# Razyehuda/Hyperparameter-GNN_unfolded-D-ADMM-main

Measured on AMD Instinct MI355X. Metric: ADMM-iters/sec (node), batch=4096 P=5 n=256 K=25; final-iter MSE vs ref, higher is better.
Workload: dtype f32; 1 GPU; DLASSO_unfolded.forward B=4096/GPU P=5 n=256 m=64 K=25 ER(p=0.5) shared graph; global_batch=4096, P=5, n=256, m=64, K=25, parallelism=batch-sharded dp1

## Files before the change

### hyperparameter-gnn_unfolded-d-admm-main_amd/csrc/dadmm_abi.cpp

```cpp

#include <hip/hip_runtime.h>
#include <stdarg.h>
#include <stdio.h>
#include <stdlib.h>
#include <string.h>

#include "../../include/dadmm.h"
#include "dadmm_internal.h"

namespace {

thread_local char g_err[512] = "";

int fail(int code, const char* fmt, ...) {
    va_list ap;
    va_start(ap, fmt);
    vsnprintf(g_err, sizeof(g_err), fmt, ap);
    va_end(ap);
    return code;
}

int ok() {
    g_err[0] = '\0';
    return DADMM_OK;
}

int hip_rc(hipError_t e, const char* what) {
    if (e != hipSuccess) return fail(DADMM_EHIP, "%s: %s", what, hipGetErrorString(e));
    return ok();
}

bool aligned16(const void* p) { return ((uintptr_t)p & 15u) == 0; }
template <typename... T>
bool all_aligned16(const T*... p) { return (... && aligned16(p)); }
template <typename... T>
bool any_null(const T*... p) { return (... || (p == nullptr)); }

int check_dims(const dadmm_dims* d) {
    if (d == nullptr) return fail(DADMM_EINVAL, "dims is NULL");
    if (d->B < 0 || d->P < 1 || d->m < 1 || d->n < 1 || d->K < 0)
        return fail(DADMM_EINVAL, "bad dims B=%d P=%d m=%d n=%d K=%d", d->B, d->P, d->m, d->n,
                    d->K);
    if (d->P > 255) return fail(DADMM_EINVAL, "P=%d > 255 agents does not fit the uint8 visit-list ids", d->P);
    if (d->variant != DADMM_VARIANT_UNFOLDED && d->variant != DADMM_VARIANT_GNN)
        return fail(DADMM_EINVAL, "unknown variant %d", d->variant);
    if (d->hyp_rows != 1 && d->hyp_rows != d->P)
        return fail(DADMM_EINVAL, "hyp_rows=%d must be 1 ('same') or P=%d ('diff')", d->hyp_rows,
                    d->P);
    if (d->graph_shared != 0 && d->graph_shared != 1)
        return fail(DADMM_EINVAL, "graph_shared must be 0 or 1");
    return DADMM_OK;
}

int n_pad_of(const dadmm_dims* d) { return 64 * dadmm::fused_nt(d->n); }
int m_pad_of(const dadmm_dims* d) { return dadmm::m_pad_of(d->m); }

int check_m(const dadmm_dims* d) {
    if (d->m > dadmm::M_MAX)
        return fail(DADMM_EUNSUPPORTED, "m=%d > %d rows per agent", d->m, dadmm::M_MAX);
    return DADMM_OK;
}

size_t align256(size_t x) { return (x + 255) & ~(size_t)255; }

int check_scratch256(const void* scratch) {
    if (((uintptr_t)scratch & 255u) != 0) return fail(DADMM_EINVAL, "scratch must be 256-byte aligned");
    return DADMM_OK;
}
int check_n4(const dadmm_dims* d, const char* who = "") {
    if ((d->n & 3) != 0) return fail(DADMM_EUNSUPPORTED, "n=%d: %sneeds n %% 4 == 0 (zero-pad n)", d->n, who);
    return DADMM_OK;
}
bool iterate_fits(const dadmm_dims* d) { return (size_t)d->B * d->P * d->n * 4 < ((size_t)1 << 31); }
int check_iterate(const dadmm_dims* d) {
    if (!iterate_fits(d)) return fail(DADMM_EUNSUPPORTED, "B*P*n*4 >= 2^31 bytes per iterate (split the batch)");
    return DADMM_OK;
}
int zero_dhyp(const dadmm_dims* d, float* dhyp, void* stream) {
    return hip_rc(hipMemsetAsync(dhyp, 0, sizeof(float) * (size_t)d->K * d->hyp_rows * 4, (hipStream_t)stream),
                  "memset");
}

template <typename Args>
void fill_args(Args& a, const dadmm_dims* d, const void* op) {
    a.A = (const float*)op;
    a.At = op ? a.A + (size_t)d->P * m_pad_of(d) * n_pad_of(d) : nullptr;
    a.B = d->B;
    a.m = d->m;
    a.n = d->n;
    a.K = d->K;
    a.hyp_rows = d->hyp_rows;
    a.variant = d->variant;
}
template <typename Args>
void fill_args_padded(Args& a, const dadmm_dims* d, const void* op) {
    fill_args(a, d, op);
    a.P = d->P;
    a.m_pad = m_pad_of(d);
    a.n_pad = n_pad_of(d);
    a.graph_shared = d->graph_shared;
}

}

extern "C" {

int dadmm_abi_version(void) { return DADMM_ABI_VERSION; }

const char* dadmm_last_error(void) { return g_err; }

size_t dadmm_operator_bytes(const dadmm_dims* d) {
    if (check_dims(d) != DADMM_OK) return 0;
    if (check_m(d) != DADMM_OK) return 0;
    return 2 * sizeof(float) * (size_t)d->P * m_pad_of(d) * (size_t)n_pad_of(d);
}

int dadmm_prepare_operator(const dadmm_dims* d, const float* A, void* op, void* stream) {
    int rc = check_dims(d);
    if (rc) return rc;
    if (A == nullptr || op == nullptr) return fail(DADMM_EINVAL, "A/op is NULL");
    if (!aligned16(op)) return fail(DADMM_EINVAL, "op workspace must be 16-byte aligned");
    if ((rc = check_m(d)) != DADMM_OK) return rc;
    const int np = n_pad_of(d);
    float* Apad = (float*)op;
    float* Atpad = Apad + (size_t)d->P * m_pad_of(d) * np;
    return hip_rc(dadmm::launch_prepare(A, Apad, Atpad, d->P, d->m, d->n, np, (hipStream_t)stream), "prepare launch");
}

}

namespace {

int check_fused_shape(const dadmm_dims* d, const uint32_t* nbr_order, int* graph, int* nt) {
    if (d->m > dadmm::M_PAD)
        return fail(DADMM_EUNSUPPORTED, "m=%d > %d rows per agent: not a fused shape", d->m,
                    dadmm::M_PAD);
    int rc = check_n4(d, "the fused kernel ");
    if (rc || (rc = check_iterate(d)) != DADMM_OK) return rc;
    if (nbr_order != nullptr && d->graph_shared)
        return fail(DADMM_EINVAL, "nbr_order needs per-sample graphs (graph_shared = 0)");
    if (nbr_order != nullptr && d->P > 8)
        return fail(DADMM_EINVAL, "nbr_order packs 4-bit agent ids: P <= 8");
    *nt = dadmm::fused_nt(d->n);
    *graph = d->graph_shared ? dadmm::GRAPH_SHARED
                             : (nbr_order ? dadmm::GRAPH_ORDERED : dadmm::GRAPH_LANE);
    return DADMM_OK;
}

void fill_fused(dadmm::FusedArgs& a, const dadmm_dims* d, const void* op, const float* b, const uint64_t* nbr,
                const uint32_t* nbr_order, const float* deg, const float* hyp, const float* y0, const float* U0,
                const float* d0, float* Y, float* U_out, int32_t* status) {
    fill_args(a, d, op);
    a.b = b;
    a.nbr = nbr;
    a.nbr_order = nbr_order;
    a.deg = deg;
    a.hyp = hyp;
    a.y0 = y0;
    a.U0 = U0;
    a.d0 = d0;
    a.Y = Y;
    a.U_out = U_out;
    a.status = status;
    a.Grec = nullptr;
    a.Urec = nullptr;
}

int forward_impl(const dadmm_dims* d, const void* op, const float* b, const uint64_t* nbr,
                 const uint32_t* nbr_order, const float* deg, const float* hyp, const float* y0,
                 const float* U0, const float* d0, float* Y, float* Grec, float* Urec,
                 float* U_out, int32_t* status, void* stream, bool rec) {
    int rc = check_dims(d);
    if (rc) return rc;
    if (d->B == 0 || d->K == 0) return ok();
    if (rec && (any_null(Grec, Urec) || !all_aligned16(Grec, Urec)))
        return fail(DADMM_EINVAL, "Grec and Urec must be non-NULL and 16-byte aligned");
    if (any_null(op, b, nbr, deg, hyp, y0, U0, d0, Y)) return fail(DADMM_EINVAL, "a required pointer is NULL");
    if (!aligned16(op)) return fail(DADMM_EINVAL, "op workspace must be 16-byte aligned");
    if (!all_aligned16(Y, y0, U0, d0, U_out))
        return fail(DADMM_EINVAL, "Y, y0, U0, d0 and U_out must be 16-byte aligned");
    int graph = 0, nt = 0;
    if ((rc = check_fused_shape(d, nbr_order, &graph, &nt)) != DADMM_OK) return rc;
    dadmm::fused_fn_ptr fn = rec ? dadmm::find_fused_rec(d->P, nt, graph) : dadmm::find_fused(d->P, nt, graph);
    if (fn == nullptr)
        return fail(DADMM_EUNSUPPORTED, "no fused kernel for P=%d n=%d (n_pad=%d)", d->P, d->n,
                    64 * nt);
    dadmm::FusedArgs a;
    fill_fused(a, d, op, b, nbr, nbr_order, deg, hyp, y0, U0, d0, Y, U_out, status);
    a.Grec = Grec;
    a.Urec = Urec;
    return hip_rc(fn(a, (hipStream_t)stream), "fused launch");
}

}

extern "C" {

int dadmm_forward(const dadmm_dims* d, const void* op, const float* b, const uint64_t* nbr,
                  const uint32_t* nbr_order, const float* deg, const float* hyp, const float* y0,
                  const float* U0, const float* d0, float* Y, float* U_out, int32_t* status,
                  void* stream) {
    return forward_impl(d, op, b, nbr, nbr_order, deg, hyp, y0, U0, d0, Y, nullptr, nullptr, U_out,
                        status, stream, false);
}

int dadmm_forward_record(const dadmm_dims* d, const void* op, const float* b, const uint64_t* nbr,
                         const uint32_t* nbr_order, const float* deg, const float* hyp,
                         const float* y0, const float* U0, const float* d0, float* Y, float* Grec,
                         float* Urec, float* U_out, int32_t* status, void* stream) {
    return forward_impl(d, op, b, nbr, nbr_order, deg, hyp, y0, U0, d0, Y, Grec, Urec, U_out,
                        status, stream, true);
}

namespace {
int device_cus() {
    int dev = 0, cus = 0;
    if (hipGetDevice(&dev) != hipSuccess ||
        hipDeviceGetAttribute(&cus, hipDeviceAttributeMultiprocessorCount, dev) != hipSuccess || cus < 1)
        cus = 256;
    return cus;
}
struct SplitPlan {
    int nt = 0, slices = 0, groups = 0, tiles = 0;
    size_t flag_bytes = 0, bytes = 0;
};
SplitPlan split_plan(const dadmm_dims* d) {
    SplitPlan sp;
    if (d == nullptr || d->B <= 0 || d->K <= 0 || d->P < 1 || d->P > 6 || d->m < 1 ||
        d->m > dadmm::M_PAD || d->n < 1 || (d->n & 3) != 0 || d->hyp_rows < 1)
        return sp;
    if (!iterate_fits(d)) return sp;
    const int nt = dadmm::fused_nt(d->n);
    if (nt != 2 && nt != 4) return sp;
    const int cus = device_cus();
    const int tiles = (d->B + dadmm::BT - 1) / dadmm::BT;
    if (2 * tiles > cus) return sp;
    const int S = 64 * nt / dadmm::SPLIT_COLS;
    int groups = cus / S;
    groups = groups < tiles ? groups : tiles;
    if (groups < 1) return sp;
    sp.nt = nt;
    sp.slices = S;
    sp.groups = groups;
    sp.tiles = tiles;
    sp.flag_bytes = ((size_t)groups * d->P * 4 * S * 4 + 4 + 255) / 256 * 256;
    sp.bytes = (size_t)groups * 2 * d->P * 4 * S * 1024;
    return sp;
}

int split_impl(const dadmm_dims* d, const void* op, const float* b, const uint64_t* nbr,
               const uint32_t* nbr_order, const float* deg, const float* hyp, const float* y0,
               const float* U0, const float* d0, float* Y, float* Grec, float* Urec, float* U_out,
               int32_t* status, void* flags, void* scratch, void* stream, bool rec) {
    int rc = check_dims(d);
    if (rc) return rc;
    if (d->B == 0 || d->K == 0) return ok();
    if (rec && (any_null(Grec, Urec) || !all_aligned16(Grec, Urec)))
        return fail(DADMM_EINVAL, "Grec and Urec must be non-NULL and 16-byte aligned");
    if (any_null(op, b, nbr, deg, hyp, y0, U0, d0, Y, flags, scratch))
        return fail(DADMM_EINVAL, "a required pointer is NULL");
    if (!all_aligned16(op, Y, y0, U0, d0, flags, scratch, U_out))
        return fail(DADMM_EINVAL, "op, Y, y0, U0, d0, U_out, flags and scratch must be 16-byte aligned");
    int graph = 0, nt = 0;
    if ((rc = check_fused_shape(d, nbr_order, &graph, &nt)) != DADMM_OK) return rc;
    const SplitPlan sp = split_plan(d);
    if (sp.groups == 0)
        return fail(DADMM_EUNSUPPORTED, "the column-split forward does not serve B=%d P=%d n=%d "
                    "(n_pad 128 or 256, P <= 6, ceil(B/16) <= CUs/2)", d->B, d->P, d->n);
    dadmm::split_fn_ptr fn = rec ? dadmm::find_split_rec(d->P, nt, graph) : dadmm::find_split(d->P, nt, graph);
    if (fn == nullptr)
        return fail(DADMM_EUNSUPPORTED, "no split kernel for P=%d n_pad=%d", d->P, 64 * nt);
    dadmm::SplitArgs sa;
    fill_fused(sa.f, d, op, b, nbr, nbr_order, deg, hyp, y0, U0, d0, Y, U_out, status);
    sa.f.Grec = Grec;
    sa.f.Urec = Urec;
    sa.xflag = (uint32_t*)flags;
    sa.xbuf = (float*)scratch;
    sa.groups = sp.groups;
    sa.tiles = sp.tiles;
    sa.spin_ticks = 20000000ull;
    return hip_rc(fn(sa, (hipStream_t)stream), "split launch");
}
}

size_t dadmm_split_scratch_bytes(const dadmm_dims* d) {
    if (d == nullptr || check_dims(d) != DADMM_OK) return 0;
    return split_plan(d).bytes;
}

size_t dadmm_split_flag_bytes(const dadmm_dims* d) {
    if (d == nullptr || check_dims(d) != DADMM_OK) return 0;
    return split_plan(d).flag_bytes;
}

int dadmm_forward_split(const dadmm_dims* d, const void* op, const float* b, const uint64_t* nbr,
                        const uint32_t* nbr_order, const float* deg, const float* hyp,
                        const float* y0, const float* U0, const float* d0, float* Y, float* U_out,
                        int32_t* status, void* flags, void* scratch, void* stream) {
    return split_impl(d, op, b, nbr, nbr_order, deg, hyp, y0, U0, d0, Y, nullptr, nullptr, U_out, status,
                      flags, scratch, stream, false);
}

int dadmm_forward_split_record(const dadmm_dims* d, const void* op, const float* b, const uint64_t* nbr,
                               const uint32_t* nbr_order, const float* deg, const float* hyp,
                               const float* y0, const float* U0, const float* d0, float* Y, float* Grec,
                               float* Urec, float* U_out, int32_t* status, void* flags, void* scratch,
                               void* stream) {
    return split_impl(d, op, b, nbr, nbr_order, deg, hyp, y0, U0, d0, Y, Grec, Urec, U_out, status,
                      flags, scratch, stream, true);
}

size_t dadmm_backward_scratch_bytes(const dadmm_dims* d) {
    if (check_dims(d) != DADMM_OK) return 0;
    const size_t nwg = ((size_t)d->B + dadmm::BT - 1) / dadmm::BT;
    const size_t bytes = sizeof(float) * nwg * (size_t)d->K * d->P * 4;
    return bytes > 0 ? bytes : 16;
}

int dadmm_backward(const dadmm_dims* d, const void* op, const uint64_t* nbr,
                   const uint32_t* nbr_order, const float* deg, const float* hyp, const float* y0,
                   const float* d0, const float* Y, const float* Grec, const float* Urec,
                   const float* gY, float* dhyp, void* scratch, void* stream) {
    int rc = check_dims(d);
    if (rc) return rc;
    if (d->K == 0) return ok();
    if (!dhyp) return fail(DADMM_EINVAL, "dhyp is NULL");
    if (d->B == 0) return zero_dhyp(d, dhyp, stream);
    if (any_null(op, nbr, deg, hyp, y0, d0, Y, Grec, Urec, gY, scratch))
        return fail(DADMM_EINVAL, "a required pointer is NULL");
    if (!all_aligned16(op, Y, y0, d0, Grec, Urec, gY, scratch))
        return fail(DADMM_EINVAL, "op, Y, y0, d0, Grec, Urec, gY and scratch must be 16-byte aligned");
    int graph = 0, nt = 0;
    if ((rc = check_fused_shape(d, nbr_order, &graph, &nt)) != DADMM_OK) return rc;
    dadmm::backward_fn_ptr fn = dadmm::find_backward(d->P, nt, graph);
    if (fn == nullptr)
        return fail(DADMM_EUNSUPPORTED, "no adjoint kernel for P=%d n=%d (n_pad=%d)", d->P, d->n,
                    64 * nt);
    dadmm::BackwardArgs a;
    fill_args(a, d, op);
    a.nbr = nbr;
    a.nbr_order = nbr_order;
    a.deg = deg;
    a.hyp = hyp;
    a.y0 = y0;
    a.d0 = d0;
    a.Y = Y;
    a.Grec = Grec;
    a.Urec = Urec;
    a.gY = gY;
    a.partial = (float*)scratch;
    if ((rc = hip_rc(fn(a, (hipStream_t)stream), "adjoint launch")) != DADMM_OK) return rc;
    const int nwg = (d->B + dadmm::BT - 1) / dadmm::BT;
    return hip_rc(dadmm::launch_backward_reduce(a.partial, dhyp, nwg, d->K, d->P, d->hyp_rows, (hipStream_t)stream),
                  "adjoint reduce launch");
}

size_t dadmm_adjoint_scratch_bytes(const dadmm_dims* d) {
    if (check_dims(d) != DADMM_OK) return 0;
    const size_t state = align256(sizeof(float) * (size_t)d->B * d->P * d->n);
    const size_t part = sizeof(float) * (size_t)dadmm::adjoint_workgroups(d->B, d->n, d->P) * d->K * d->P * 4;
    return 3 * state + align256(part > 0 ? part : 16);
}

int dadmm_adjoint(const dadmm_dims* d, const void* op, const int32_t* visit_ptr,
                  const uint8_t* visit_q, const float* deg, const float* hyp, const float* y0,
                  const float* d0, const float* Y, const float* Grec, const float* Urec,
                  const float* gY, float* dhyp, void* scratch, void* stream) {
    int rc = check_dims(d);
    if (rc) return rc;
    if (d->K == 0) return ok();
    if (!dhyp) return fail(DADMM_EINVAL, "dhyp is NULL");
    if (d->B == 0) return zero_dhyp(d, dhyp, stream);
    if (any_null(op, visit_ptr, visit_q, deg, hyp, y0, d0, Y, Grec, Urec, gY, scratch))
        return fail(DADMM_EINVAL, "a required pointer is NULL");
    if (!all_aligned16(op, Y, y0, d0, Grec, Urec, gY))
        return fail(DADMM_EINVAL, "op, Y, y0, d0, Grec, Urec and gY must be 16-byte aligned");
    if ((rc = check_scratch256(scratch)) != DADMM_OK || (rc = check_m(d)) != DADMM_OK ||
        (rc = check_n4(d)) != DADMM_OK || (rc = check_iterate(d)) != DADMM_OK)
        return rc;
    if (dadmm::adjoint_lds_bytes(d->P) > 160 * 1024 || dadmm::gnn_gram_lds(m_pad_of(d)) > 160 * 1024)
        return fail(DADMM_EUNSUPPORTED, "P=%d / m=%d: the adjoint's LDS tiles do not fit", d->P, d->m);
    const size_t state = align256(sizeof(float) * (size_t)d->B * d->P * d->n);
    char* base = (char*)scratch;
    dadmm::AdjArgs a{};
    fill_args_padded(a, d, op);
    a.vptr = visit_ptr;
    a.vq = visit_q;
    a.deg = deg;
    a.hyp = hyp;
    a.y0 = y0;
    a.d0 = d0;
    a.Y = Y;
    a.Grec = Grec;
    a.Urec = Urec;
    a.gY = gY;
    a.yb = (float*)base;
    a.Ub = (float*)(base + state);
    a.Gb = (float*)(base + 2 * state);
    a.partial = (float*)(base + 3 * state);
    return hip_rc(dadmm::launch_adjoint(a, dhyp, (hipStream_t)stream), "adjoint launch");
}

namespace {

int gnn_common(const dadmm_dims* d, const void* op, dadmm::GnnArgs* a) {
    int rc = check_dims(d);
    if (rc || (rc = check_m(d)) != DADMM_OK || (rc = check_n4(d)) != DADMM_OK ||
        (rc = check_iterate(d)) != DADMM_OK)
        return rc;
    *a = dadmm::GnnArgs{};
    fill_args_padded(*a, d, op);
    return DADMM_OK;
}

}

size_t dadmm_gnn_flag_bytes(int32_t K) {
    return K < 0 ? 0 : (size_t)GNN_FLAG_WORDS(K) * 4;
}

int dadmm_gnn_begin(const dadmm_dims* d, const void* op, const float* b, const float* y0,
                    const float* U0, float* Atb, int32_t* flags, void* stream) {
    dadmm::GnnArgs a;
    int rc = gnn_common(d, op, &a);
    if (rc) return rc;
    if (!flags) return fail(DADMM_EINVAL, "flags is NULL");
    if (d->B == 0) return hip_rc(dadmm::gnn_launch_zero(flags, GNN_FLAG_WORDS(d->K), (hipStream_t)stream), "zero launch");
    if (any_null(op, b, y0, U0, Atb)) return fail(DADMM_EINVAL, "a required pointer is NULL");
    if (!all_aligned16(op, y0, U0, Atb))
        return fail(DADMM_EINVAL, "op, y0, U0 and Atb must be 16-byte aligned");
    a.b = b;
    a.U = U0;
    a.flags = flags;
    if ((rc = hip_rc(dadmm::gnn_launch_zero(flags, GNN_FLAG_WORDS(d->K), (hipStream_t)stream), "zero launch")) ||
        (rc = hip_rc(dadmm::gnn_launch_check0(a, y0, (hipStream_t)stream), "check0 launch")))
        return rc;
    return hip_rc(dadmm::gnn_launch_gram(a, 0, nullptr, Atb, 1, (hipStream_t)stream), "Atb launch");
}

int dadmm_gnn_gram(const dadmm_dims* d, const void* op, int32_t k, float* const* yptr,
                   const int32_t* flags, const float* x, float* out, void* stream) {
    dadmm::GnnArgs a;
    int rc = gnn_common(d, op, &a);
    if (rc) return rc;
    if (d->B == 0) return ok();
    if (!op || !out || (x == nullptr && (yptr == nullptr || flags == nullptr)))
        return fail(DADMM_EINVAL, "a required pointer is NULL");
    if (x == nullptr && (k < 0 || k >= d->K)) return fail(DADMM_EINVAL, "k=%d outside [0, K)", k);
    if (!all_aligned16(op, out, x))
        return fail(DADMM_EINVAL, "op, x and out must be 16-byte aligned");
    if (dadmm::gnn_gram_lds(a.m_pad) > 160 * 1024)
        return fail(DADMM_EUNSUPPORTED, "m=%d too large for the gram tile", d->m);
    a.yptr = yptr;
    a.flags = const_cast<int32_t*>(flags);
    return hip_rc(dadmm::gnn_launch_gram(a, k, x, out, 0, (hipStream_t)stream), "gram launch");
}

int dadmm_gnn_gram_acc(const dadmm_dims* d, const void* op, const float* x, float* out, const float* addend,
                       void* stream) {
    dadmm::GnnArgs a;
    int rc = gnn_common(d, op, &a);
    if (rc) return rc;
    if (d->B == 0) return ok();
    if (any_null(op, out, x)) return fail(DADMM_EINVAL, "a required pointer is NULL");
    if (!all_aligned16(op, out, x))
        return fail(DADMM_EINVAL, "op, x and out must be 16-byte aligned");
    if (dadmm::gnn_gram_lds(a.m_pad) > 160 * 1024)
        return fail(DADMM_EUNSUPPORTED, "m=%d too large for the gram tile", d->m);
    if (!aligned16(addend)) return fail(DADMM_EINVAL, "addend must be 16-byte aligned");
    a.acc_add = addend;
    return hip_rc(dadmm::gnn_launch_gram(a, 0, x, out, 2, (hipStream_t)stream), "gram launch");
}

int dadmm_gnn_step(const dadmm_dims* d, int32_t k, const int32_t* visit_ptr, const uint8_t* visit_q,
                   const float* deg, const float* hyp_k, float* const* yptr, const float* AtAy,
                   const float* Atb, const float* U, const float* D, float* U_next, float* D_next,
                   float* G, int32_t* flags, void* stream) {
    dadmm::GnnArgs a;
    int rc = gnn_common(d, nullptr, &a);
    if (rc) return rc;
    if (k < 0 || k >= d->K) return fail(DADMM_EINVAL, "k=%d outside [0, K)", k);
    if (d->B == 0) return ok();
    if (any_null(visit_ptr, visit_q, deg, hyp_k, yptr, AtAy, Atb, U, D, U_next, D_next, G, flags))
        return fail(DADMM_EINVAL, "a required pointer is NULL");
    if (!all_aligned16(AtAy, Atb, U, D, G, U_next, D_next))
        return fail(DADMM_EINVAL, "AtAy, Atb, U, D, U_next, D_next and G must be 16-byte aligned");
    a.vptr = visit_ptr;
    a.vq = visit_q;
    a.deg = deg;
// ... 814 lines not shown
```

### hyperparameter-gnn_unfolded-d-admm-main_amd/csrc/dadmm_internal.h

```cpp
#pragma once

#include <hip/hip_runtime.h>
#include <stdint.h>

namespace dadmm {

constexpr int BT = 16;
constexpr int M_PAD = 64;
constexpr int M_MAX = 1024;
__host__ __device__ constexpr int m_pad_of(int m) { return (m + M_PAD - 1) / M_PAD * M_PAD; }
constexpr int FUSED_WAVES = 8;

struct FusedArgs {
    const float* A;
    const float* At;
    const float* b;
    const uint64_t* nbr;
    const uint32_t* nbr_order;
    const float* deg;
    const float* hyp;
    const float* y0;
    const float* U0;
    const float* d0;
    float* Y;
    float* U_out;
    int32_t* status;
    float* Grec;
    float* Urec;
    int B, m, n, K, hyp_rows, variant;
};

typedef hipError_t (*fused_fn_ptr)(const FusedArgs&, hipStream_t);

enum { GRAPH_SHARED = 0, GRAPH_LANE = 1, GRAPH_ORDERED = 2 };
fused_fn_ptr find_fused(int P, int nt, int graph);
fused_fn_ptr find_fused_rec(int P, int nt, int graph);

constexpr int SPLIT_COLS = 64;
struct SplitArgs {
    FusedArgs f;
    float* xbuf;
    uint32_t* xflag;
    int groups;
    int tiles;
    uint64_t spin_ticks;
};
typedef hipError_t (*split_fn_ptr)(const SplitArgs&, hipStream_t);
split_fn_ptr find_split(int P, int nt, int graph);
split_fn_ptr find_split_rec(int P, int nt, int graph);

struct BackwardArgs {
    const float* A;
    const float* At;
    const uint64_t* nbr;
    const uint32_t* nbr_order;
    const float* deg;
    const float* hyp;
    const float* y0;
    const float* d0;
    const float* Y;
    const float* Grec;
    const float* Urec;
    const float* gY;
    float* partial;
    int B, m, n, K, hyp_rows, variant;
};
typedef hipError_t (*backward_fn_ptr)(const BackwardArgs&, hipStream_t);
backward_fn_ptr find_backward(int P, int nt, int graph);
hipError_t launch_backward_reduce(const float* partial, float* dhyp, int nwg, int K, int P, int H,
                                  hipStream_t stream);

struct AdjArgs {
    const float* A;
    const float* At;
    const int32_t* vptr;
    const uint8_t* vq;
    const float* deg;
    const float* hyp;
    const float* y0;
    const float* d0;
    const float* Y;
    const float* Grec;
    const float* Urec;
    const float* gY;
    float* yb;
    float* Ub;
    float* Gb;
    float* partial;
    int B, P, m, m_pad, n, n_pad, K, hyp_rows, variant, graph_shared;
};
size_t adjoint_lds_bytes(int P);
int adjoint_workgroups(int B, int n, int P);
int adjoint_waves(int P);
hipError_t launch_adjoint(const AdjArgs& a, float* dhyp, hipStream_t st);

#define GNN_F_Y0 0
#define GNN_F_UBAD(k) (1 + 5 * (k))
#define GNN_F_GBAD(k) (2 + 5 * (k))
#define GNN_F_YNB(k) (3 + 5 * (k))
#define GNN_F_YNB_OPT(k) (4 + 5 * (k))
#define GNN_F_UNB_OPT(k) (5 + 5 * (k))
#define GNN_FLAG_WORDS(K) (5 * (K) + 4)

struct GnnArgs {
    const float* A;
    const float* At;
    const float* b;
    const int32_t* vptr;
    const uint8_t* vq;
    const float* deg;
    const float* hyp;
    float* const* yptr;
    const float* yk;
    const float* AtAy;
    const float* Atb;
    const float* U;
    const float* D;
    float* U_next;
    float* D_next;
    float* G;
    int32_t* flags;
    int32_t* status;
    int B, P, m, m_pad, n, n_pad, K, hyp_rows, variant, graph_shared;
    const float* acc_add;
};
struct GnnGrads {
    const float* gy1;
    const float* gU1;
    const float* gd1;
    float* gy;
    float* gU;
    float* gd;
    float* gAtAy;
    float* ghyp;
    const float* ghyp_add;
    const float* hz;
    float* hdz;
    float hmax[4];
};
hipError_t gnn_launch_zero(int32_t* p, int words, hipStream_t st);
hipError_t gnn_launch_check0(const GnnArgs& a, const float* y0, hipStream_t st);
hipError_t gnn_launch_gram(const GnnArgs& a, int k, const float* x_raw, float* out, int mode,
                           hipStream_t st);
hipError_t gnn_launch_step(const GnnArgs& a, int k, hipStream_t st);
hipError_t gnn_launch_finish(const GnnArgs& a, hipStream_t st);
hipError_t gnn_launch_step_backward(const GnnArgs& a, int k, const GnnGrads& gg, hipStream_t st);
size_t gnn_gram_lds(int m_pad);

struct TiledArgs {
    const float* A;
    const float* At;
    const float* b;
    const int32_t* vptr;
    const uint8_t* vq;
    const float* deg;
    const float* hyp;
    const float* y0;
    const float* U0;
    const float* d0;
    float* Y;
    float* Ubuf[2];
    float* delta;
    float* R;
    float* U_out;
    int32_t* status;
    int B, P, m, m_pad, n, n_pad, K, hyp_rows, variant, graph_shared;
    float* Grec;
    float* Urec;
};
size_t tiled_lds_bytes(int n_pad, int m_pad);
hipError_t launch_tiled(const TiledArgs& a, hipStream_t stream);
bool stream_applies(const TiledArgs& a);
hipError_t launch_stream(const TiledArgs& a, hipStream_t stream);

struct LossArgs {
    const float* Y;
    const float* label;
    float* partial;
    float* losses;
    float* out;
    int32_t* flags;
    int K, P, n, n_store;
    int64_t rows;
};
size_t loss_scratch_floats(int K, int64_t rows, int n);
hipError_t launch_loss(const LossArgs& a, hipStream_t st);
hipError_t launch_loss_grad(const LossArgs& a, const float* gout, float* dY, hipStream_t st);

#define HYPER_EPI_BIAS 0
#define HYPER_EPI_GCN 1
#define HYPER_EPI_HEAD 2
#define HYPER_EPI_GCN_TRAIN 3
#define HYPER_EPI_GCN_BWD 4
struct HyperArgs {
    const float* x1;
    const float* x2;
    int ld1, ld2, K1;
    const float* W;
    int ldw;
    const float* bias;
    float* y;
    int ldy;
    int rows, K, N;
    int B, P, S_t;
    const float* ahat;
    int ahat_per_sample;
    const float* bn_mean;
    const float* bn_var;
    const float* bn_w;
    const float* bn_b;
    float bn_eps, slope;
    int H;
    float maxv[4];
    int splits;
    size_t split_stride;
    int gm, gn;
    float* save_m;
    float* save_mean;
    float* save_var;
    float drop_p;
    uint64_t seed;
    int site;
    const float* addend;
    int ld_add, raw;
    float* part;
    int bn_eval;
    int kwave;
};

__host__ __device__ inline uint32_t drop_hash(uint64_t seed, int site, uint32_t row, uint32_t col) {
    uint64_t z = seed ^ ((uint64_t)(uint32_t)site << 56) ^ ((uint64_t)row << 20) ^ (uint64_t)col;
    z += 0x9E3779B97F4A7C15ull;
    z = (z ^ (z >> 30)) * 0xBF58476D1CE4E5B9ull;
    z = (z ^ (z >> 27)) * 0x94D049BB133111EBull;
    z ^= z >> 31;
    return (uint32_t)(z >> 32);
}
__host__ __device__ inline uint32_t drop_threshold(float p) {
    const double t = (double)p * 4294967296.0;
    return t >= 4294967295.0 ? 0xFFFFFFFFu : (uint32_t)t;
}
hipError_t launch_hyper(HyperArgs a, int epi, hipStream_t st);
int hyper_linear_gcn_dx(int32_t P, int32_t rows, int32_t K, int32_t N, const float* x, int32_t ldx, const float* W,
                        const float* addend, int32_t ld_add, float* y, int32_t ldy, void* stream);
int hyper_linear_splits(int rows, int K, int N);
struct RowNormArgs {
    const float* x;
    const float* weight;
    const float* bias;
    float* y;
    int rows, C, act;
    float eps, slope;
    int nsum;
    size_t sum_stride;
    const float* pre_bias;
    float drop_p;
    uint64_t seed;
    int site;
    float* xd;
};
struct RowNormBwdArgs {
    const float* dy;
    const float* xd;
    const float* weight;
    const float* bias;
    float* dx;
    float* part;
    int rows, C, act;
    float eps, slope, drop_p;
    uint64_t seed;
    int site;
};
hipError_t launch_rownorm_bwd(const RowNormBwdArgs& a, hipStream_t st);
constexpr int ROWNORM_BWD_ROWS = 8;
struct GcnBwdArgs {
    const float* dy;
    const float* m;
    const float* mean;
    const float* var;
    const float* gamma;
    const float* ahat;
    int ahat_per_sample;
    float* dz;
    float* part;
    int B, P, N;
    float eps, slope, drop_p;
    uint64_t seed;
    int site;
    int bn_eval;
};
hipError_t launch_gcn_bwd(const GcnBwdArgs& a, hipStream_t st);
int gcn_train_impl(int32_t B, int32_t P, int32_t K, int32_t N, const float* x1, int32_t ld1, int32_t K1,
                   const float* x2, int32_t ld2, const float* W, int32_t ldw, const float* addend, int32_t ld_add,
                   const float* bias, const float* ahat, int32_t ahat_per_sample, const float* bn_weight,
                   const float* bn_bias, float bn_eps, float slope, float drop_p, uint64_t seed, int32_t site,
                   float* y, int32_t ldy, float* m_out, float* mean_out, float* var_out,
                   const float* bn_running_mean, const float* bn_running_var, void* stream);

struct TailArgs {
    int B, H;
    int D[3];
    const float* x0;
    const float* W[3];
    const float* bias[3];
    const float* lnw[2];
    const float* lnb[2];
    float eps[2], slope[2], drop[2];
    uint64_t seed;
    int site0;
    float* xd[2];
    float* y[2];
    float* z;
    float* hyp;
    float maxv[4];
    const float* dz;
    const float* Wt[3];
    float* dv[2];
    float* part[2];
    float* dx0;
};
size_t tail_lds_bytes(const TailArgs& a, bool bwd);
hipError_t launch_tail(const TailArgs& a, bool bwd, hipStream_t st);

constexpr int BN_MAX_LAYERS = 8;
struct BnRunArgs {
    int layers, iters, B, P;
    int width[BN_MAX_LAYERS];
    int col0[BN_MAX_LAYERS + 1];
    float* rmean[BN_MAX_LAYERS];
    float* rvar[BN_MAX_LAYERS];
    int64_t* tracked[BN_MAX_LAYERS];
    const float* mean[BN_MAX_LAYERS];
    const float* var[BN_MAX_LAYERS];
    int64_t block_stride;
    const double* w;
    double decay;
    double* part;
    int splits;
};
// ... 95 lines not shown
```

Baseline: 188.3 million ADMM-iters/s.

## Add warp-specialized fused forward kernel splitting matrix and update roles

Adds a new fused forward kernel in which four waves run the A/At GEMMs with MFMA and a register ring of prefetched fragments, while the other four waves run the elementwise ADMM update and consensus step. The two roles hand off data through LDS and are kept in lockstep by barriers. The goal is to overlap matrix and update work across waves on each SIMD, so that GEMM latency is hidden behind update work. It is enabled by default for P<=5, n_pad=256 and a shared graph, with an environment variable to opt out. It adds barrier-coupled scheduling complexity, and the specialization is limited to that shape.

```diff
diff --git a/hyperparameter-gnn_unfolded-d-admm-main_amd/csrc/dadmm_abi.cpp b/hyperparameter-gnn_unfolded-d-admm-main_amd/csrc/dadmm_abi.cpp
--- a/hyperparameter-gnn_unfolded-d-admm-main_amd/csrc/dadmm_abi.cpp
+++ b/hyperparameter-gnn_unfolded-d-admm-main_amd/csrc/dadmm_abi.cpp
@@ -166,6 +166,8 @@
     a.Urec = nullptr;
 }
 
+constexpr bool FUSED_ROLES_DEFAULT = true;
+
 int forward_impl(const dadmm_dims* d, const void* op, const float* b, const uint64_t* nbr,
                  const uint32_t* nbr_order, const float* deg, const float* hyp, const float* y0,
                  const float* U0, const float* d0, float* Y, float* Grec, float* Urec,
@@ -185,6 +187,12 @@
     if (fn == nullptr)
         return fail(DADMM_EUNSUPPORTED, "no fused kernel for P=%d n=%d (n_pad=%d)", d->P, d->n,
                     64 * nt);
+    if (!rec) {
+        const char* fenv = getenv("DADMM_FUSED_FORM");
+        const bool roles = fenv != nullptr ? strcmp(fenv, "roles") == 0 : FUSED_ROLES_DEFAULT;
+        dadmm::fused_fn_ptr rfn = roles ? dadmm::find_fused_roles(d->P, nt, graph) : nullptr;
+        if (rfn != nullptr) fn = rfn;
+    }
     dadmm::FusedArgs a;
     fill_fused(a, d, op, b, nbr, nbr_order, deg, hyp, y0, U0, d0, Y, U_out, status);
     a.Grec = Grec;
diff --git a/hyperparameter-gnn_unfolded-d-admm-main_amd/csrc/dadmm_fused_roles.hip b/hyperparameter-gnn_unfolded-d-admm-main_amd/csrc/dadmm_fused_roles.hip
--- /dev/null
+++ b/hyperparameter-gnn_unfolded-d-admm-main_amd/csrc/dadmm_fused_roles.hip
@@ -0,0 +1,410 @@
+
+#include <hip/hip_runtime.h>
+#include <stdint.h>
+
+#include <type_traits>
+
+#include "dadmm_internal.h"
+#include "dadmm_consensus.h"
+#include "dadmm_device.h"
+
+namespace dadmm {
+
+template <int P>
+struct Roles {
+    static constexpr int NP = 256;
+    static constexpr int NB = NP / 16;
+    static constexpr int MP = M_PAD;
+    static constexpr int YS = NP + 8;
+    static constexpr int RS = MP + 8;
+    static constexpr int GS = NP + 8;
+    static constexpr int RD = P == 5 ? 20 : 16;
+    static constexpr int NF = 32 * P;
+    static constexpr int G1A = (P - 1) / 2;
+    static constexpr int G1B = P - G1A;
+    static constexpr int LDS_FLOATS = P * BT * YS + P * BT * RS + 2 * BT * GS;
+    static_assert((16 * P) % RD == 0, "ring slots must line up at the GEMM2 / GEMM1 boundary");
+};
+
+template <int V>
+using ic = std::integral_constant<int, V>;
+
+__device__ __forceinline__ void pin() { __builtin_amdgcn_sched_barrier(0); }
+__device__ __forceinline__ void stage_barrier() {
+    pin();
+    __syncthreads();
+    pin();
+}
+
+template <int P>
+__device__ __forceinline__ void roles_matrix(const FusedArgs& a, float* __restrict__ lds, const int w) {
+    using C = Roles<P>;
+    constexpr int NP = C::NP, NB = C::NB, MP = C::MP, YS = C::YS, RS = C::RS, GS = C::GS;
+    constexpr int RD = C::RD, NF = C::NF, G1A = C::G1A, G1B = C::G1B;
+    float* __restrict__ Ylds = lds;
+    float* __restrict__ Rlds = lds + P * BT * YS;
+    float* __restrict__ Glds = Rlds + P * BT * RS;
+
+    const int lane = threadIdx.x & 63;
+    const int j = lane & 15;
+    const int h = lane >> 4;
+    const int s = blockIdx.x * BT + j;
+    const bool sv = s < a.B;
+    const int m = a.m;
+
+    const rsrc_t rA = make_rsrc(a.A, (uint32_t)(P * MP * NP * 4));
+    const rsrc_t rAt = make_rsrc(a.At, (uint32_t)(P * MP * NP * 4));
+
+    f32x4 bseed[P];
+#pragma unroll
+    for (int p = 0; p < P; ++p) {
+        f32x4 v;
+#pragma unroll
+        for (int r = 0; r < 4; ++r) {
+            const int mi = 16 * w + 4 * h + r;
+            v[r] = (sv && mi < m) ? -a.b[((size_t)s * P + p) * m + mi] : 0.0f;
+        }
+        bseed[p] = v;
+    }
+
+    const uint32_t voffA = (uint32_t)(((16 * w + j) * NP + 4 * h) * 4);
+    const uint32_t voffAt = (uint32_t)(((64 * w + j) * MP + 4 * h) * 4);
+    const float* brow = Ylds + j * YS + 4 * h;
+    uint32_t vA = voffA, vAt = voffAt;
+
+    f32x4 ring[RD];
+    auto frag_load = [&](int i) {
+        if (i < 16 * P) {
+            const int p = i / 16, t = (i % 16) / 4, tt = i % 4;
+            ring[i % RD] = bload4(rAt, vAt + 64 * t, (uint32_t)((p * NP + 16 * tt) * MP * 4));
+        } else {
+            int ii = i - 16 * P, p, t;
+            if (ii < 16 * G1A) {
+                t = ii / (G1A > 0 ? G1A : 1);
+                p = ii % (G1A > 0 ? G1A : 1);
+            } else {
+                ii -= 16 * G1A;
+                t = ii / G1B;
+                p = G1A + ii % G1B;
+            }
+            ring[i % RD] = bload4(rA, vA + 64 * t, (uint32_t)(p * MP * NP * 4));
+        }
+    };
+
+    auto gemm1 = [&](auto p0_, auto cnt_, auto base_) {
+        constexpr int P0 = decltype(p0_)::value, CNT = decltype(cnt_)::value, BASE = decltype(base_)::value;
+        if constexpr (CNT > 0) {
+            f32x4 acc[CNT];
+            f32x4 bring[2][CNT];
+#pragma unroll
+            for (int i = 0; i < CNT; ++i) {
+                acc[i] = bseed[P0 + i];
+                bring[0][i] = *(const f32x4*)(brow + (P0 + i) * BT * YS);
+            }
+#pragma unroll
+            for (int t = 0; t < NB; ++t) {
+                if (t + 1 < NB) {
+#pragma unroll
+                    for (int i = 0; i < CNT; ++i)
+                        bring[(t + 1) & 1][i] = *(const f32x4*)(brow + (P0 + i) * BT * YS + 16 * (t + 1));
+                }
+#pragma unroll
+                for (int r = 0; r < 4; ++r)
+#pragma unroll
+                    for (int i = 0; i < CNT; ++i)
+                        acc[i] = mfma4(ring[(BASE + t * CNT + i) % RD][r], bring[t & 1][i][r], acc[i]);
+#pragma unroll
+                for (int i = 0; i < CNT; ++i) frag_load((BASE + t * CNT + i + RD) % NF);
+                pin();
+            }
+#pragma unroll
+            for (int i = 0; i < CNT; ++i)
+                *(f32x4*)(Rlds + ((P0 + i) * BT + j) * RS + 16 * w + 4 * h) = acc[i];
+        }
+    };
+
+    f32x4 rvb[2][MP / 16];
+    auto load_r = [&](int p) {
+#pragma unroll
+        for (int t = 0; t < MP / 16; ++t)
+            rvb[p & 1][t] = *(const f32x4*)(Rlds + (p * BT + j) * RS + 4 * h + 16 * t);
+    };
+    auto gemm2 = [&](auto p_) {
+        constexpr int p = decltype(p_)::value;
+        if constexpr (p + 1 < P) load_r(p + 1);
+        f32x4 gc[4];
+#pragma unroll
+        for (int tt = 0; tt < 4; ++tt) gc[tt] = (f32x4){0.0f, 0.0f, 0.0f, 0.0f};
+#pragma unroll
+        for (int t = 0; t < MP / 16; ++t) {
+#pragma unroll
+            for (int r = 0; r < 4; ++r)
+#pragma unroll
+                for (int tt = 0; tt < 4; ++tt)
+                    gc[tt] = mfma4(ring[(16 * p + 4 * t + tt) % RD][r], rvb[p & 1][t][r], gc[tt]);
+#pragma unroll
+            for (int tt = 0; tt < 4; ++tt) frag_load((16 * p + 4 * t + tt + RD) % NF);
+            pin();
+        }
+#pragma unroll
+        for (int tt = 0; tt < 4; ++tt)
+            *(f32x4*)(Glds + ((p & 1) * BT + j) * GS + 16 * (4 * w + tt) + 4 * h) = gc[tt];
+    };
+    auto gemm2_all = [&](auto self, auto p_) -> void {
+        constexpr int p = decltype(p_)::value;
+        if constexpr (p < P) {
+            gemm2(p_);
+            stage_barrier();
+            self(self, ic<p + 1>{});
+        }
+    };
+
+#pragma unroll
+    for (int i = 0; i < RD; ++i) frag_load(16 * P + i);
+    __syncthreads();
+
+    gemm1(ic<0>{}, ic<G1A>{}, ic<16 * P>{});
+    gemm1(ic<G1A>{}, ic<G1B>{}, ic<16 * P + 16 * G1A>{});
+    stage_barrier();
+
+    for (int k = 0; k < a.K; ++k) {
+        vA = fresh(voffA);
+        vAt = fresh(voffAt);
+        load_r(0);
+        gemm2_all(gemm2_all, ic<0>{});
+        if (k + 1 < a.K) {
+            gemm1(ic<0>{}, ic<G1A>{}, ic<16 * P>{});
+            stage_barrier();
+            gemm1(ic<G1A>{}, ic<G1B>{}, ic<16 * P + 16 * G1A>{});
+            stage_barrier();
+        } else {
+            __syncthreads();
+            __syncthreads();
+        }
+    }
+}
+
+template <int P>
+__device__ __forceinline__ void roles_update(const FusedArgs& a, float* __restrict__ lds, const int u) {
+    using C = Roles<P>;
+    constexpr int NP = C::NP, MP = C::MP, YS = C::YS, RS = C::RS, GS = C::GS;
+    constexpr int T2 = 4;
+    constexpr int E = T2 * 4;
+    float* __restrict__ Ylds = lds;
+    float* __restrict__ Glds = lds + P * BT * YS + P * BT * RS;
+    (void)NP; (void)MP;
+
+    const int lane = threadIdx.x & 63;
+    const int j = lane & 15;
+    const int h = lane >> 4;
+    const int s = blockIdx.x * BT + j;
+    const int n = a.n, B = a.B;
+    const uint32_t state_bytes = (uint32_t)((size_t)B * P * n * 4);
+
+    uint32_t msk[P];
+    float dg[P];
+#pragma unroll
+    for (int p = 0; p < P; ++p) {
+        msk[p] = __builtin_amdgcn_readfirstlane((uint32_t)a.nbr[p]);
+        dg[p] = a.deg[p];
+    }
+
+    float U[P][E], D[P][E];
+    uint32_t ymag = 0, umag = 0;
+    {
+        const rsrc_t ry = make_rsrc(a.y0, state_bytes);
+        const rsrc_t ru = make_rsrc(a.U0, state_bytes);
+        const rsrc_t rd = make_rsrc(a.d0, state_bytes);
+#pragma unroll
+        for (int tt = 0; tt < T2; ++tt) {
+            const int nb = u * T2 + tt;
+            const int n0 = nb * 16 + 4 * h;
+#pragma unroll
+            for (int p = 0; p < P; ++p) {
+                const uint32_t off = n0 < n ? (uint32_t)(((s * P + p) * n + n0) * 4) : 0x80000000u;
+                const f32x4 vy = bload4(ry, off, 0);
+                const f32x4 vu = bload4(ru, off, 0);
+                const f32x4 vd = bload4(rd, off, 0);
+#pragma unroll
+                for (int r = 0; r < 4; ++r) {
+                    ymag = max(ymag, __float_as_uint(vy[r]) & 0x7fffffffu);
+                    umag = max(umag, __float_as_uint(vu[r]) & 0x7fffffffu);
+                    U[p][4 * tt + r] = vu[r];
+                    D[p][4 * tt + r] = vd[r];
+                }
+                *(f32x4*)(Ylds + (p * BT + j) * YS + n0) = vy;
+            }
+            ymag = fresh(ymag);
+            umag = fresh(umag);
+            compiler_fence();
+        }
+    }
+    __syncthreads();
+
+    uint32_t status = (ymag >= 0x7f800000u ? 1u : 0u) | (umag >= 0x7f800000u ? 2u : 0u);
+    {
+        bool bad_h = false;
+        const int nh = a.K * a.hyp_rows * 4;
+        for (int i = threadIdx.x - 256; i < nh; i += 256) bad_h |= !finitef(a.hyp[i]);
+        status |= bad_h ? 8u : 0u;
+    }
+    float mf[P][P];
+#pragma unroll
+    for (int q = 0; q < P; ++q)
+#pragma unroll
+        for (int p = 0; p < P; ++p) mf[q][p] = 0.0f;
+    {
+        bool asym = false;
+#pragma unroll
+        for (int q = 0; q < P; ++q)
+#pragma unroll
+            for (int p = q + 1; p < P; ++p) {
+                const bool e1 = (msk[q] >> p) & 1u, e2 = (msk[p] >> q) & 1u;
+                asym |= e1 != e2;
+                mf[q][p] = __uint_as_float(__builtin_amdgcn_readfirstlane(e1 ? 0x3f800000u : 0u));
+            }
+        status |= asym ? 16u : 0u;
+    }
+    const uint32_t voffY = (uint32_t)((s * P * n + 4 * h) * 4);
+    const float dlim = a.variant != 0 ? GNN_DELTA_LIMIT : __builtin_inff();
+    __syncthreads();
+
+    for (int k = 0; k < a.K; ++k) {
+        float al[P], ta[P], rh[P], et[P];
+#pragma unroll
+        for (int p = 0; p < P; ++p) {
+            const cfloat* hp = (const cfloat*)a.hyp + ((size_t)k * a.hyp_rows + (a.hyp_rows == 1 ? 0 : p)) * 4;
+            al[p] = hp[0]; ta[p] = hp[1]; rh[p] = hp[2]; et[p] = hp[3];
+        }
+        float gclip, vclip;
+        iter_clips(a.variant, k, gclip, vclip);
+        const rsrc_t rY = make_rsrc(a.Y + (size_t)k * B * P * n, state_bytes);
+        const uint32_t vY = fresh(voffY);
+        uint32_t gmag = 0;
+        __syncthreads();
+
+#pragma unroll
+        for (int p = 0; p < P; ++p) {
+            const float* __restrict__ Gp = Glds + ((p & 1) * BT + j) * GS;
+            f32x4 gpb[2], ykb[2];
+            gpb[0] = *(const f32x4*)(Gp + u * T2 * 16 + 4 * h);
+            ykb[0] = *(const f32x4*)(Ylds + (p * BT + j) * YS + u * T2 * 16 + 4 * h);
+#pragma unroll
+            for (int tt = 0; tt < T2; ++tt) {
+                const int nb = u * T2 + tt;
+                const int n0 = nb * 16 + 4 * h;
+                if (tt + 1 < T2) {
+                    gpb[(tt + 1) & 1] = *(const f32x4*)(Gp + n0 + 16);
+                    ykb[(tt + 1) & 1] = *(const f32x4*)(Ylds + (p * BT + j) * YS + n0 + 16);
+                }
+                compiler_fence();
+                const f32x4 gp = gpb[tt & 1];
+                const f32x4 yk = ykb[tt & 1];
+                f32x4 yn;
+#pragma unroll
+                for (int r = 0; r < 4; ++r) {
+                    const int e = 4 * tt + r;
+                    const float yv = yk[r];
+                    const float st = sign_times(yv, ta[p]);
+                    float gr = gp[r];
+                    gr = gr + st;
+                    gr = gr + U[p][e] * dg[p];
+                    gr = gr + D[p][e] * rh[p];
+                    gmag = max(gmag, __float_as_uint(gr) & 0x7fffffffu);
+                    gr = mclamp(gr, -gclip, gclip);
+                    float v = yv - al[p] * gr;
+                    v = mclamp(v, -vclip, vclip);
+                    yn[r] = v;
+                }
+                gmag = fresh(gmag);
+                *(f32x4*)(Ylds + (p * BT + j) * YS + n0) = yn;
+                bstore4<16>(yn, rY, n0 < n ? vY : 0x80000000u, (uint32_t)((p * n + nb * 16) * 4));
+            }
+            __syncthreads();
+        }
+        status |= gmag > 0x7f800000u ? 4u : 0u;
+
+        if (k + 1 < a.K || a.U_out != nullptr) {
+#pragma unroll
+            for (int tt = 0; tt < T2; ++tt) {
+                const int n0 = (u * T2 + tt) * 16 + 4 * h;
+                compiler_fence();
+                f32x4 yv[P];
+#pragma unroll
+                for (int p = 0; p < P; ++p) yv[p] = *(const f32x4*)(Ylds + (p * BT + j) * YS + n0);
+#pragma unroll
+                for (int r = 0; r < 4; ++r) {
+                    const int e = 4 * tt + r;
+                    float yy[P][1], dd[P][1];
+#pragma unroll
+                    for (int p = 0; p < P; ++p) {
+                        float y = yv[p][r];
+                        if (e > 0) asm volatile("" : "+v"(y) : "v"(U[P - 1][e - 1]));
+                        yy[p][0] = y;
+                    }
+                    consensus_fma<P>(yy, dd, mf);
+#pragma unroll
+                    for (int p = 0; p < P; ++p) {
+                        const float d = mclamp(dd[p][0], -dlim, dlim);
+                        U[p][e] = mclamp(U[p][e] + d * et[p], -vclip, vclip);
+                        D[p][e] = d;
+                    }
+                }
+            }
+        }
+        __syncthreads();
+    }
+
+    if (a.U_out != nullptr) {
+        const rsrc_t rU = make_rsrc(a.U_out, state_bytes);
+#pragma unroll
+        for (int tt = 0; tt < T2; ++tt) {
+            const int n0 = (u * T2 + tt) * 16 + 4 * h;
+            if (n0 < n) {
+#pragma unroll
+                for (int p = 0; p < P; ++p) {
+                    const f32x4 v = {U[p][4 * tt], U[p][4 * tt + 1], U[p][4 * tt + 2], U[p][4 * tt + 3]};
+                    bstore4(v, rU, (uint32_t)(((s * P + p) * n + n0) * 4), 0);
+                }
+            }
+        }
+    }
+    if (a.status != nullptr) {
+        uint32_t wst = status;
+#pragma unroll
+        for (int off = 32; off >= 1; off >>= 1) wst |= __shfl_xor(wst, off);
+        if (lane == 0 && wst) atomicOr((unsigned int*)a.status, wst);
+    }
+}
+
+template <int P>
+__global__ __launch_bounds__(FUSED_WAVES * 64) void fused_roles_kernel(FusedArgs a) {
+    __shared__ __attribute__((aligned(16))) float lds[Roles<P>::LDS_FLOATS];
+    static_assert(FUSED_WAVES == 8, "one matrix wave and one update wave per SIMD");
+    const int w = __builtin_amdgcn_readfirstlane(threadIdx.x >> 6);
+    if (w < 4)
+        roles_matrix<P>(a, lds, w);
+    else
+        roles_update<P>(a, lds, w - 4);
+}
+
+template <int P>
+static hipError_t launch_roles(const FusedArgs& a, hipStream_t stream) {
+    const int grid = (a.B + BT - 1) / BT;
+    hipLaunchKernelGGL((fused_roles_kernel<P>), dim3(grid), dim3(FUSED_WAVES * 64), 0, stream, a);
+    return hipGetLastError();
+}
+
+fused_fn_ptr find_fused_roles(int P, int nt, int graph) {
+    if (nt != 4 || graph != GRAPH_SHARED) return nullptr;
+    switch (P) {
+        case 1: return &launch_roles<1>;
+        case 2: return &launch_roles<2>;
+        case 3: return &launch_roles<3>;
+        case 4: return &launch_roles<4>;
+        case 5: return &launch_roles<5>;
+        default: return nullptr;
+    }
+}
+
+}
diff --git a/hyperparameter-gnn_unfolded-d-admm-main_amd/csrc/dadmm_internal.h b/hyperparameter-gnn_unfolded-d-admm-main_amd/csrc/dadmm_internal.h
--- a/hyperparameter-gnn_unfolded-d-admm-main_amd/csrc/dadmm_internal.h
+++ b/hyperparameter-gnn_unfolded-d-admm-main_amd/csrc/dadmm_internal.h
@@ -35,6 +35,7 @@
 enum { GRAPH_SHARED = 0, GRAPH_LANE = 1, GRAPH_ORDERED = 2 };
 fused_fn_ptr find_fused(int P, int nt, int graph);
 fused_fn_ptr find_fused_rec(int P, int nt, int graph);
+fused_fn_ptr find_fused_roles(int P, int nt, int graph);
 
 constexpr int SPLIT_COLS = 64;
 struct SplitArgs {
```

Measured after the change: 193.5 million ADMM-iters/s, median of 6. 2.7% higher.
